# 0xJchen/HanabiZero

Measured on NVIDIA B200. Metric: mcts_simulations_per_sec, higher is better.
Workload: dtype f32

## Files before the change

hanabizero_b200/csrc/hz_rowchain.cu:

```cuda
#include <cuda.h>
#include <cuda_fp16.h>

#include <stdlib.h>
#include <string.h>

#include "hz_common.cuh"

namespace hz {

constexpr int kBM = 128, kBK = 64, kF = 512, kH = 256;
constexpr int kKB = kBM * kBK * 2;
constexpr int kActBytes = kBM * kF * 2;
constexpr int kWSlot = 256 * kBK * 2;
constexpr int kWSlots = 3;
constexpr int kOffW = kActBytes, kOffAux = kOffW + kWSlots * kWSlot;
constexpr int kAuxBytes = 128 + 1024;
constexpr int kRowSmem = kOffAux + kAuxBytes + 1024;
constexpr int kEpiWarps = 16, kEpiThreads = kEpiWarps * 32, kRowThreads = 64 + kEpiThreads;
constexpr int kMaxPhases = 10, kMaps = 10;
constexpr int kMapX0 = 7, kMapState = 8, kMapOut = 9;
constexpr unsigned kSpin = 1u << 26;

struct RowJob {
  int32_t map, n0, batch, num_k, a_kb, n, half;
  int32_t relu, dst_kb;
  int32_t res, res_off;
  int32_t gout, gb;
  int32_t kb1;
  const __half* bias;
};
struct RowPhase {
  int32_t njobs, after;
  int32_t a_wait, res_load;
  RowJob job[2];
};
struct alignas(64) RowParams {
  CUtensorMap maps[kMaps];
  RowPhase phase[kMaxPhases];
  int32_t n_phases, rows, row_blocks, p3;
  const __half* x0; int64_t ld_x0;
  const __half* w1a_t;
  __half* state;
  __half* out;
  unsigned long long* trace;
};

namespace rc {

__device__ __forceinline__ uint32_t smem_u32(const void* p) { return (uint32_t)__cvta_generic_to_shared(p); }
__device__ __forceinline__ void mbar_init(uint32_t bar, uint32_t count) {
  asm volatile("mbarrier.init.shared::cta.b64 [%0], %1;" ::"r"(bar), "r"(count) : "memory");
}
__device__ __forceinline__ void mbar_expect_tx(uint32_t bar, uint32_t bytes) {
  asm volatile("mbarrier.arrive.expect_tx.shared::cta.b64 _, [%0], %1;" ::"r"(bar), "r"(bytes) : "memory");
}
__device__ __forceinline__ void mbar_arrive(uint32_t bar) {
  asm volatile("mbarrier.arrive.shared::cta.b64 _, [%0];" ::"r"(bar) : "memory");
}
__device__ __forceinline__ void mbar_wait(uint32_t bar, uint32_t parity) {
  uint32_t done = 0;
  for (unsigned spin = 0; !done; ++spin) {
    asm volatile(
        "{\n\t.reg .pred p;\n\t"
        "mbarrier.try_wait.parity.shared::cta.b64 p, [%1], %2;\n\t"
        "selp.u32 %0, 1, 0, p;\n\t}"
        : "=r"(done) : "r"(bar), "r"(parity) : "memory");
    if (spin > kSpin) __trap();
  }
}
__device__ __forceinline__ void tma_load_3d(uint32_t dst, const CUtensorMap* map, uint32_t bar, int c0, int c1, int c2) {
  asm volatile(
      "cp.async.bulk.tensor.3d.shared::cta.global.mbarrier::complete_tx::bytes [%0], [%1, {%3, %4, %5}], [%2];"
      ::"r"(dst), "l"(map), "r"(bar), "r"(c0), "r"(c1), "r"(c2) : "memory");
}
__device__ __forceinline__ void tma_store_3d(const CUtensorMap* map, uint32_t src, int c0, int c1, int c2) {
  asm volatile(
      "cp.async.bulk.tensor.3d.global.shared::cta.bulk_group [%0, {%2, %3, %4}], [%1];"
      ::"l"(map), "r"(src), "r"(c0), "r"(c1), "r"(c2) : "memory");
}
__device__ __forceinline__ void tma_commit() { asm volatile("cp.async.bulk.commit_group;" ::: "memory"); }
__device__ __forceinline__ void tma_wait_read_all() { asm volatile("cp.async.bulk.wait_group.read 0;" ::: "memory"); }
__device__ __forceinline__ void tma_wait_all() { asm volatile("cp.async.bulk.wait_group 0;" ::: "memory"); }
__device__ __forceinline__ void tma_wait_all_but_last() { asm volatile("cp.async.bulk.wait_group 1;" ::: "memory"); }
__device__ __forceinline__ void tma_prefetch_desc(const CUtensorMap* map) {
  asm volatile("prefetch.tensormap [%0];" ::"l"(map) : "memory");
}
__device__ __forceinline__ void tc_fence_before() { asm volatile("tcgen05.fence::before_thread_sync;" ::: "memory"); }
__device__ __forceinline__ void tc_fence_after() { asm volatile("tcgen05.fence::after_thread_sync;" ::: "memory"); }
__device__ __forceinline__ void tc_commit(uint32_t bar) {
  asm volatile("tcgen05.commit.cta_group::1.mbarrier::arrive::one.shared::cluster.b64 [%0];" ::"r"(bar) : "memory");
}
__device__ __forceinline__ void tc_mma_f16(uint32_t tmem_d, uint64_t desc_a, uint64_t desc_b, uint32_t idesc,
                                           uint32_t accumulate) {
  asm volatile(
      "{\n\t.reg .pred p;\n\t"
      "setp.ne.b32 p, %4, 0;\n\t"
      "tcgen05.mma.cta_group::1.kind::f16 [%0], %1, %2, %3, p;\n\t}"
      ::"r"(tmem_d), "l"(desc_a), "l"(desc_b), "r"(idesc), "r"(accumulate) : "memory");
}
__device__ __forceinline__ void tc_ld16(uint32_t taddr, uint32_t* r) {
  asm volatile(
      "tcgen05.ld.sync.aligned.32x32b.x16.b32 "
      "{%0, %1, %2, %3, %4, %5, %6, %7, %8, %9, %10, %11, %12, %13, %14, %15}, [%16];"
      : "=r"(r[0]), "=r"(r[1]), "=r"(r[2]), "=r"(r[3]), "=r"(r[4]), "=r"(r[5]), "=r"(r[6]), "=r"(r[7]),
        "=r"(r[8]), "=r"(r[9]), "=r"(r[10]), "=r"(r[11]), "=r"(r[12]), "=r"(r[13]), "=r"(r[14]), "=r"(r[15])
      : "r"(taddr) : "memory");
}
__device__ __forceinline__ void tc_wait_ld() { asm volatile("tcgen05.wait::ld.sync.aligned;" ::: "memory"); }

__device__ __forceinline__ uint64_t umma_desc_k128(uint32_t saddr) {
  uint64_t d = 0;
  d |= (uint64_t)((saddr & 0x3ffffu) >> 4);
  d |= (uint64_t)1 << 16;
  d |= (uint64_t)(1024 >> 4) << 32;
  d |= (uint64_t)1 << 46;
  d |= (uint64_t)2 << 61;
  return d;
}
__device__ __forceinline__ bool elect_one() {
  uint32_t pred;
  asm volatile(
      "{\n\t.reg .pred p;\n\t"
      "elect.sync _|p, 0xffffffff;\n\t"
      "selp.u32 %0, 1, 0, p;\n\t}"
      : "=r"(pred));
  return pred != 0;
}
__device__ __forceinline__ void st_shared_v4(uint32_t addr, uint4 v) {
  asm volatile("st.shared.v4.u32 [%0], {%1, %2, %3, %4};" ::"r"(addr), "r"(v.x), "r"(v.y), "r"(v.z), "r"(v.w) : "memory");
}
__device__ __forceinline__ uint4 ld_shared_v4(uint32_t addr) {
  uint4 v;
  asm volatile("ld.shared.v4.u32 {%0, %1, %2, %3}, [%4];" : "=r"(v.x), "=r"(v.y), "=r"(v.z), "=r"(v.w) : "r"(addr) : "memory");
  return v;
}
__device__ __forceinline__ uint32_t act_off(int r, int ch) {
  return (uint32_t)((ch >> 3) * kKB + (r >> 3) * 1024 + (r & 7) * 128 + ((((ch & 7) ^ (r & 7))) << 4));
}
__device__ __forceinline__ void stamp(const RowParams& P, int phase, int slot) {
  if (P.trace) {
    unsigned long long t;
    asm volatile("mov.u64 %0, %%globaltimer;" : "=l"(t));
    P.trace[((size_t)blockIdx.x * kMaxPhases + phase) * 4 + slot] = t;
  }
}

}

using namespace rc;

__global__ void __launch_bounds__(kRowThreads, 1) k_row_chain(const __grid_constant__ RowParams P) {
  extern __shared__ uint8_t smem_raw[];
  const uint32_t base = (smem_u32(smem_raw) + 1023u) & ~1023u;
  const uint32_t act = base, wbase = base + kOffW, aux = base + kOffAux;
  auto w_full = [&](int s) { return aux + 8u * s; };
  auto w_empty = [&](int s) { return aux + 8u * (kWSlots + s); };
  auto acc_full = [&](int h) { return aux + 8u * (2 * kWSlots + h); };
  const uint32_t ready0 = aux + 8u * (2 * kWSlots + 2), ready1 = ready0 + 8u;
  const uint32_t a_full = ready1 + 8u;
  const uint32_t res_full = a_full + 8u;
  const uint32_t tmem_slot = res_full + 8u;
  const uint32_t sbias = aux + 128u;
  const int warp = __shfl_sync(0xffffffffu, (int)(threadIdx.x >> 5), 0), lane = threadIdx.x & 31;

  if (warp == 0 && lane == 0) {
    for (int s = 0; s < kWSlots; ++s) { mbar_init(w_full(s), 1); mbar_init(w_empty(s), 1); }
    mbar_init(acc_full(0), 1);
    mbar_init(acc_full(1), 1);
    mbar_init(ready0, kEpiWarps);
    mbar_init(ready1, kEpiWarps);
    mbar_init(a_full, 1);
    mbar_init(res_full, 1);
    asm volatile("fence.mbarrier_init.release.cluster;" ::: "memory");
    for (int m = 0; m < kMaps; ++m) tma_prefetch_desc(&P.maps[m]);
  }
  if (warp == 1) {
    asm volatile("tcgen05.alloc.cta_group::1.sync.aligned.shared::cta.b32 [%0], %1;" ::"r"(tmem_slot), "n"(512) : "memory");
    asm volatile("tcgen05.relinquish_alloc_permit.cta_group::1.sync.aligned;" ::: "memory");
  }
  tc_fence_before();
  __syncthreads();
  tc_fence_after();
  uint32_t tmem_base;
  asm volatile("ld.shared.u32 %0, [%1];" : "=r"(tmem_base) : "r"(tmem_slot) : "memory");

  if (warp == 0) {
    const bool leader = elect_one();
    uint32_t slot = 0, e_par = 0xffffffffu;
    for (int rb = blockIdx.x; rb < P.row_blocks; rb += gridDim.x) {
      for (int ph = 0; ph < P.n_phases; ++ph) {
        const RowPhase& F = P.phase[ph];
        for (int j = 0; j < F.njobs; ++j) {
          const RowJob& J = F.job[j];
          const uint32_t bytes = (uint32_t)J.n * (kBK * 2);
          for (int kb = 0; kb < J.num_k; ++kb) {
            mbar_wait(w_empty(slot), (e_par >> slot) & 1u);
            e_par ^= 1u << slot;
            if (leader) {
              mbar_expect_tx(w_full(slot), bytes);
              tma_load_3d(wbase + slot * kWSlot, &P.maps[J.map], w_full(slot), kb * kBK, J.n0, J.batch);
            }
            __syncwarp();
            if (++slot == kWSlots) slot = 0;
          }
        }
      }
    }
  } else if (warp == 1) {
    const bool leader = elect_one();
    uint32_t slot = 0, f_par = 0, r0_par = 0, r1_par = 0, af_par = 0;
    bool first_rb = true;
    for (int rb = blockIdx.x; rb < P.row_blocks; rb += gridDim.x) {
      for (int ph = 0; ph < P.n_phases; ++ph) {
        const RowPhase& F = P.phase[ph];
        mbar_wait(ready0, r0_par);
        r0_par ^= 1u;
        tc_fence_after();
        bool got1 = false;
        auto need_all = [&]() {
          mbar_wait(ready1, r1_par);
          r1_par ^= 1u;
          if (F.a_wait) {
            mbar_wait(a_full, af_par);
            af_par ^= 1u;
          }
          tc_fence_after();
          got1 = true;
        };
        if (leader && first_rb) stamp(P, ph, 0);
        for (int j = 0; j < F.njobs; ++j) {
          const RowJob& J = F.job[j];
          const uint32_t d_tmem = tmem_base + (uint32_t)J.half * 256u;
          const uint32_t idesc = (1u << 4) | ((uint32_t)(J.n >> 3) << 17) | ((uint32_t)(kBM >> 4) << 24);
          uint64_t da = umma_desc_k128(act + (uint32_t)J.a_kb * kKB);
          for (int kb = 0; kb < J.num_k; ++kb) {
            if (!got1 && (j > 0 || kb >= J.kb1)) need_all();
            mbar_wait(w_full(slot), (f_par >> slot) & 1u);
            f_par ^= 1u << slot;
            tc_fence_after();
            if (leader) {
              const uint64_t dw = umma_desc_k128(wbase + slot * kWSlot);
#pragma unroll
              for (int k16 = 0; k16 < kBK / 16; ++k16) {
                tc_mma_f16(d_tmem, da + (uint64_t)(2 * k16), dw + (uint64_t)(2 * k16), idesc, (kb | k16) != 0);
              }
              tc_commit(w_empty(slot));
            }
            __syncwarp();
            da += (uint64_t)(kKB >> 4);
            if (++slot == kWSlots) slot = 0;
          }
          if (leader) tc_commit(acc_full(J.half));
          __syncwarp();
        }
        if (!got1) need_all();
        if (leader && first_rb) stamp(P, ph, 1);
      }
      first_rb = false;
    }
  } else {
    const int q = warp & 3, part = (warp - 2) >> 2, et = threadIdx.x - 64;
    const int rloc = q * 32 + lane;
    uint32_t a_par = 0;
    bool first_rb = true;
    auto load_tile = [&](int map, int rb_, uint32_t bar) {
      mbar_expect_tx(bar, kActBytes);
#pragma unroll
      for (int kb = 0; kb < kF / kBK; ++kb) tma_load_3d(act + kb * kKB, &P.maps[map], bar, kb * kBK, rb_ * kBM, 0);
    };
    uint32_t rf_par = 0;
    if (et == 0) load_tile(kMapX0, blockIdx.x, a_full);
    __syncwarp();
    if (lane == 0) { mbar_arrive(ready0); mbar_arrive(ready1); }
    for (int rb = blockIdx.x; rb < P.row_blocks; rb += gridDim.x) {
      const int row = rb * kBM + rloc;
      const bool live = row < P.rows;
      for (int ph = 0; ph < P.n_phases; ++ph) {
        const RowPhase& F = P.phase[ph];
        if (et == 0) tma_wait_read_all();
        asm volatile("bar.sync 1, %0;" ::"n"(kEpiThreads) : "memory");
        {
          const int j = et >> 8, col = et & 255;
          if (j < F.njobs && col < F.job[j].n) {
            const unsigned short bv = __half_as_ushort(F.job[j].bias[col]);
            asm volatile("st.shared.u16 [%0], %1;" ::"r"(sbias + 2u * et), "h"(bv) : "memory");
          }
        }
        const __half* crow[2] = {nullptr, nullptr};
        uint4 ef0 = make_uint4(0, 0, 0, 0), ef1 = ef0;
#pragma unroll
        for (int j = 0; j < 2; ++j) {
          if (j >= F.njobs) continue;
          const RowJob& J = F.job[j];
          if (J.res == 1 && live) {
            const uint4* oh = reinterpret_cast<const uint4*>(P.x0 + (size_t)row * P.ld_x0 + kF);
            int a = -1;
#pragma unroll
            for (int v = 0; v < 4; ++v) {
              const uint4 w = oh[v];
              const uint32_t u[4] = {w.x, w.y, w.z, w.w};
#pragma unroll
              for (int t = 0; t < 4; ++t) {
                if ((u[t] & 0xffffu) == 0x3c00u) a = v * 8 + t * 2;
                if ((u[t] >> 16) == 0x3c00u) a = v * 8 + t * 2 + 1;
              }
            }
            if (a >= 0) crow[j] = P.w1a_t + (size_t)a * kF + J.res_off;
          } else if (J.res == 2 && live) {
            crow[j] = P.x0 + (size_t)row * P.ld_x0 + J.res_off;
          }
          if (j == 0 && crow[0]) {
            const int c0 = ((part * (J.n >> 4)) >> 2) * 16;
            ef0 = __ldg(reinterpret_cast<const uint4*>(crow[0] + c0));
            ef1 = __ldg(reinterpret_cast<const uint4*>(crow[0] + c0 + 8));
          }
        }
        asm volatile("bar.sync 1, %0;" ::"n"(kEpiThreads) : "memory");
        for (int j = 0; j < F.njobs; ++j) {
          const int h = F.job[j].half;
          mbar_wait(acc_full(h), (a_par >> h) & 1u);
          a_par ^= 1u << h;
        }
        tc_fence_after();
        if (et == 0 && first_rb) stamp(P, ph, 2);
        if (F.res_load) {
          if (et == 0) load_tile(kMapX0, rb, res_full);
          mbar_wait(res_full, rf_par);
          rf_par ^= 1u;
        }
        bool any_store = false;
#pragma unroll
        for (int j = 0; j < 2; ++j) {
          if (j >= F.njobs) continue;
          const RowJob& J = F.job[j];
          const int n16 = J.n >> 4;
          const int c_begin = ((part * n16) >> 2) * 16, c_end = (((part + 1) * n16) >> 2) * 16;
          const uint32_t t_addr = tmem_base + (uint32_t)J.half * 256u + ((uint32_t)(q * 32) << 16);
          const uint32_t sb = sbias + (uint32_t)j * 512u;
          const __half* cr = crow[j];
          const int res = J.res, relu = J.relu, dst_kb = J.dst_kb, res_off = J.res_off;
          any_store |= J.gout != 0;
          auto fetch_res = [&](int c, uint4& e0, uint4& e1) {
            if (res == 3) {
              const int ch = res_off * 8 + (c >> 3);
              e0 = ld_shared_v4(act + act_off(rloc, ch));
              e1 = ld_shared_v4(act + act_off(rloc, ch + 1));
            } else if (cr) {
              e0 = __ldg(reinterpret_cast<const uint4*>(cr + c));
              e1 = __ldg(reinterpret_cast<const uint4*>(cr + c + 8));
            }
          };
          auto emit = [&](const uint32_t (&r)[16], const uint4& e0, const uint4& e1, int c) {
            const uint4 b0 = ld_shared_v4(sb + 2u * (uint32_t)c), b1 = ld_shared_v4(sb + 2u * (uint32_t)c + 16u);
            float v[16];
            const __half2* h0 = reinterpret_cast<const __half2*>(&b0);
            const __half2* h1 = reinterpret_cast<const __half2*>(&b1);
#pragma unroll
            for (int t = 0; t < 4; ++t) {
              const float2 f0 = __half22float2(h0[t]), f1 = __half22float2(h1[t]);
              v[2 * t] = __uint_as_float(r[2 * t]) + f0.x;
              v[2 * t + 1] = __uint_as_float(r[2 * t + 1]) + f0.y;
              v[8 + 2 * t] = __uint_as_float(r[8 + 2 * t]) + f1.x;
              v[8 + 2 * t + 1] = __uint_as_float(r[8 + 2 * t + 1]) + f1.y;
            }
            if (res != 0) {
              const __half2* g0 = reinterpret_cast<const __half2*>(&e0);
              const __half2* g1 = reinterpret_cast<const __half2*>(&e1);
#pragma unroll
              for (int t = 0; t < 4; ++t) {
                const float2 x0 = __half22float2(g0[t]), x1 = __half22float2(g1[t]);
                v[2 * t] += x0.x; v[2 * t + 1] += x0.y; v[8 + 2 * t] += x1.x; v[8 + 2 * t + 1] += x1.y;
              }
            }
            uint4 o0, o1;
            __half2* p0 = reinterpret_cast<__half2*>(&o0);
            __half2* p1 = reinterpret_cast<__half2*>(&o1);
#pragma unroll
            for (int t = 0; t < 4; ++t) {
              p0[t] = __floats2half2_rn(v[2 * t], v[2 * t + 1]);
              p1[t] = __floats2half2_rn(v[8 + 2 * t], v[8 + 2 * t + 1]);
            }
            if (relu) {
              const __half2 z = __float2half2_rn(0.0f);
#pragma unroll
              for (int t = 0; t < 4; ++t) { p0[t] = __hmax2(p0[t], z); p1[t] = __hmax2(p1[t], z); }
            }
            if (dst_kb >= 0) {
              const int ch = dst_kb * 8 + (c >> 3);
              st_shared_v4(act + act_off(rloc, ch), o0);
              st_shared_v4(act + act_off(rloc, ch + 1), o1);
            }
          };
          uint32_t ra[16], rb2[16];
          uint4 ea0 = ef0, ea1 = ef1, eb0 = make_uint4(0, 0, 0, 0), eb1 = eb0;
          if (j == 1 || res == 3) {
            ea0 = ea1 = make_uint4(0, 0, 0, 0);
            fetch_res(c_begin, ea0, ea1);
          }
          tc_ld16(t_addr + (uint32_t)c_begin, ra);
          for (int c = c_begin; c < c_end; c += 32) {
            tc_wait_ld();
            const bool more1 = c + 16 < c_end;
            if (more1) {
              tc_ld16(t_addr + (uint32_t)(c + 16), rb2);
              if (res != 0) fetch_res(c + 16, eb0, eb1);
            }
            emit(ra, ea0, ea1, c);
            if (more1) {
              tc_wait_ld();
              if (c + 32 < c_end) {
                tc_ld16(t_addr + (uint32_t)(c + 32), ra);
                if (res != 0) fetch_res(c + 32, ea0, ea1);
              }
              emit(rb2, eb0, eb1, c + 16);
            }
          }
          if (j == 0) {
            asm volatile("fence.proxy.async.shared::cta;" ::: "memory");
            tc_fence_before();
            __syncwarp();
            if (lane == 0) mbar_arrive(ready0);
          }
        }
        if (any_store || F.after != 0) {
          asm volatile("fence.proxy.async.shared::cta;" ::: "memory");
          asm volatile("bar.sync 1, %0;" ::"n"(kEpiThreads) : "memory");
          if (et == 0) {
            for (int j = 0; j < F.njobs; ++j) {
              const RowJob& J = F.job[j];
              if (J.gout == 1 && j == 0) {
                for (int kb = 0; kb < kF / kBK; ++kb) tma_store_3d(&P.maps[kMapState], act + kb * kKB, kb * kBK, rb * kBM, 0);
              } else if (J.gout == 2) {
                for (int i = 0; i * kBK < P.p3; ++i)
                  tma_store_3d(&P.maps[kMapOut], act + (J.dst_kb + i) * kKB, i * kBK, rb * kBM, J.gb);
              }
            }
            if (any_store) tma_commit();
            if (F.after == 1) {
              tma_wait_all_but_last();
              tma_wait_read_all();
              asm volatile("fence.proxy.async;" ::: "memory");
              load_tile(kMapState, rb, a_full);
            } else if (F.after == 2 && rb + (int)gridDim.x < P.row_blocks) {
              tma_wait_read_all();
              load_tile(kMapX0, rb + gridDim.x, a_full);
            }
          }
        }
        if (et == 0 && first_rb) stamp(P, ph, 3);
        asm volatile("fence.proxy.async.shared::cta;" ::: "memory");
        tc_fence_before();
        __syncwarp();
        if (lane == 0) mbar_arrive(ready1);
      }
      first_rb = false;
    }
  }

  if (threadIdx.x == 64) tma_wait_all();
  tc_fence_before();
  __syncthreads();
  if (warp == 1) {
    asm volatile("tcgen05.dealloc.cta_group::1.sync.aligned.b32 %0, %1;" ::"r"(tmem_base), "n"(512) : "memory");
  }
}

typedef CUresult (*EncodeTiledFn)(CUtensorMap*, CUtensorMapDataType, cuuint32_t, void*, const cuuint64_t*,
                                  const cuuint64_t*, const cuuint32_t*, const cuuint32_t*, CUtensorMapInterleave,
                                  CUtensorMapSwizzle, CUtensorMapL2promotion, CUtensorMapFloatOOBfill);

static EncodeTiledFn encode_fn() {
  static EncodeTiledFn fn = [] {
    void* p = nullptr;
    cudaDriverEntryPointQueryResult q;
    if (cudaGetDriverEntryPoint("cuTensorMapEncodeTiled", &p, cudaEnableDefault, &q) != cudaSuccess ||
        q != cudaDriverEntryPointSuccess) {
      p = nullptr;
    }
    cudaGetLastError();
    return (EncodeTiledFn)p;
  }();
  return fn;
}

static bool make_w_map(CUtensorMap* map, const void* ptr, int64_t k, int64_t n, int64_t batch, int64_t ld, int box_n) {
  EncodeTiledFn fn = encode_fn();
  if (!fn) return false;
  cuuint64_t dims[3] = {(cuuint64_t)k, (cuuint64_t)n, (cuuint64_t)batch};
  cuuint64_t strides[2] = {(cuuint64_t)ld * 2, (cuuint64_t)(n * ld) * 2};
  cuuint32_t box[3] = {(cuuint32_t)kBK, (cuuint32_t)box_n, 1};
  cuuint32_t estr[3] = {1, 1, 1};
  return fn(map, CU_TENSOR_MAP_DATA_TYPE_FLOAT16, 3, const_cast<void*>(ptr), dims, strides, box, estr,
            CU_TENSOR_MAP_INTERLEAVE_NONE, CU_TENSOR_MAP_SWIZZLE_128B, CU_TENSOR_MAP_L2_PROMOTION_L2_256B,
            CU_TENSOR_MAP_FLOAT_OOB_FILL_NONE) == CUDA_SUCCESS;
}

}

using namespace hz;

struct hz_rowchain {
  int device = 0, grid = 0, sms = 0;
  RowParams params;
  unsigned long long* trace = nullptr;
};

extern "C" {
#pragma GCC visibility push(default)

int hz_rowchain_create(hz_rowchain** out, int device, const hz_rowchain_weights* w, int rows, const void* x0,
                       int64_t ld_x0, void* state, void* out_logits) {
  if (!out || !w || rows <= 0 || !x0 || !state || !out_logits) { set_error("hz_rowchain_create: bad argument"); return HZ_ERR_ARG; }
  if (w->state_cols != kF || w->head_cols != kH || w->onehot_cols != 32 || w->logit_cols <= 0 || w->logit_cols > 256 ||
      w->logit_cols % 16 || ld_x0 < kF + 32 || ld_x0 % 8 || w->ld_w1 < kF + 32 || w->ld_w1 % 8) {
    set_error("hz_rowchain_create: this executor is built for state 512 / heads 256 / one-hot 32 / logits <= 256 (multiple of 16)");
    return HZ_ERR_ARG;
  }
  const void* ptrs[] = {w->w1, w->w1a_t, w->b1, w->w2, w->b2, w->w3, w->b3, w->wh1, w->bh1, w->wb2, w->bb2,
                        w->wa2, w->ba2, w->wb3, w->bb3, x0, state, out_logits};
  for (const void* p : ptrs) {
    if (!p || ((uintptr_t)p & 15)) { set_error("hz_rowchain_create: null or unaligned pointer"); return HZ_ERR_ARG; }
  }
  DeviceGuard dg(device);
  if (!dg.ok) { set_error("hz_rowchain_create: cannot select device %d", device); return HZ_ERR_CUDA; }
  if (!encode_fn()) { set_error("hz_rowchain_create: cuTensorMapEncodeTiled unavailable"); return HZ_ERR_CUDA; }
  hz_rowchain* e = new hz_rowchain;
  e->device = device;
  RowParams& P = e->params;
  memset(&P, 0, sizeof(P));
  const int p3 = w->logit_cols;
  bool ok = make_w_map(&P.maps[0], w->w1, kF, kF, 1, w->ld_w1, 256) &&
            make_w_map(&P.maps[1], w->w2, kF, kF, 1, kF, 256) &&
            make_w_map(&P.maps[2], w->w3, kF, kF, 1, kF, 256) &&
            make_w_map(&P.maps[3], w->wh1, kF, 3 * kH, 1, kF, 256) &&
            make_w_map(&P.maps[4], w->wb2, kH, kH, 3, kH, 256) &&
            make_w_map(&P.maps[5], w->wa2, kH, kH, 1, kH, 256) &&
            make_w_map(&P.maps[6], w->wb3, kH, p3, 3, kH, p3) &&
            make_w_map(&P.maps[kMapX0], x0, kF, rows, 1, ld_x0, kBM) &&
            make_w_map(&P.maps[kMapState], state, kF, rows, 1, kF, kBM) &&
            make_w_map(&P.maps[kMapOut], out_logits, p3, rows, 3, p3, kBM);
  if (!ok) { delete e; set_error("hz_rowchain_create: cuTensorMapEncodeTiled failed"); return HZ_ERR_CUDA; }
  const __half *b1 = (const __half*)w->b1, *b2 = (const __half*)w->b2, *b3 = (const __half*)w->b3,
               *bh1 = (const __half*)w->bh1, *bb2 = (const __half*)w->bb2, *ba2 = (const __half*)w->ba2,
               *bb3 = (const __half*)w->bb3;
  auto job = [](int map, int n0, int batch, int num_k, int a_kb, int n, int half, const __half* bias, int relu,
                int dst_kb, int res = 0, int res_off = 0, int gout = 0, int gb = 0) {
    RowJob j;
    memset(&j, 0, sizeof(j));
    j.map = map; j.n0 = n0; j.batch = batch; j.num_k = num_k; j.a_kb = a_kb; j.n = n; j.half = half;
    j.bias = bias; j.relu = relu; j.dst_kb = dst_kb; j.res = res; j.res_off = res_off; j.gout = gout; j.gb = gb;
    return j;
  };
  int np = 0;
  auto phase = [&](int after, RowJob j0, const RowJob* j1 = nullptr, int a_wait = 0) {
    RowPhase& F = P.phase[np++];
    F.after = after; F.njobs = j1 ? 2 : 1; F.job[0] = j0; F.a_wait = a_wait;
    if (j1) F.job[1] = *j1;
  };
  RowJob t;
  t = job(0, 256, 0, 8, 0, 256, 1, b1 + 256, 1, 4, 1, 256);  phase(0, job(0, 0, 0, 8, 0, 256, 0, b1, 1, 0, 1, 0), &t, 1);
  t = job(1, 256, 0, 8, 0, 256, 1, b2 + 256, 1, 4);          phase(0, job(1, 0, 0, 8, 0, 256, 0, b2, 1, 0), &t);
  t = job(2, 256, 0, 8, 0, 256, 1, b3 + 256, 1, 4, 3, 4, 1);
  phase(0, job(2, 0, 0, 8, 0, 256, 0, b3, 1, 0, 3, 0, 1), &t);
  P.phase[np - 1].res_load = 1;
  t = job(3, 512, 0, 8, 0, 256, 1, bh1 + 512, 1, 4);         phase(0, job(3, 256, 0, 8, 0, 256, 0, bh1 + 256, 1, 0), &t);
  t = job(4, 0, 2, 4, 4, 256, 1, bb2 + 512, 1, 4);           phase(0, job(4, 0, 1, 4, 0, 256, 0, bb2 + 256, 1, 0), &t);
  t = job(6, 0, 1, 4, 4, p3, 1, bb3 + p3, 0, 4, 0, 0, 2, 1);
  phase(1, job(6, 0, 0, 4, 0, p3, 0, bb3, 0, 0, 0, 0, 2, 0), &t);
  phase(0, job(3, 0, 0, 8, 0, 256, 0, bh1, 1, 0), nullptr, 1);
  phase(0, job(4, 0, 0, 4, 0, 256, 1, bb2, 1, 4));
  phase(0, job(5, 0, 0, 4, 4, 256, 0, ba2, 1, 0, 3, 0));
  phase(2, job(6, 0, 2, 4, 0, p3, 1, bb3 + 2 * p3, 0, 4, 0, 0, 2, 2));
  for (int p = 0; p < np; ++p) {
    RowPhase& F = P.phase[p];
    F.job[0].kb1 = 0;
    F.job[1].kb1 = 0;
    if (p == 0 || F.a_wait) continue;
    const RowJob& A = P.phase[p - 1].job[0];
    RowJob& J = F.job[0];
    if (J.half != A.half || A.dst_kb < 0 || P.phase[p - 1].after != 0) continue;
    const int w0 = (A.n + kBK - 1) / kBK;
    int k = 0;
    while (k < J.num_k && J.a_kb + k >= A.dst_kb && J.a_kb + k < A.dst_kb + w0) ++k;
    J.kb1 = k;
  }
  P.n_phases = np;
  P.rows = rows;
  P.row_blocks = (rows + kBM - 1) / kBM;
  P.p3 = p3;
  P.x0 = (const __half*)x0;
  P.ld_x0 = ld_x0;
  P.w1a_t = (const __half*)w->w1a_t;
  P.state = (__half*)state;
  P.out = (__half*)out_logits;
  cudaError_t err = cudaFuncSetAttribute(k_row_chain, cudaFuncAttributeMaxDynamicSharedMemorySize, kRowSmem);
  cudaDeviceProp prop;
  if (err == cudaSuccess) err = cudaGetDeviceProperties(&prop, device);
  if (err != cudaSuccess) { delete e; return fail_cuda(err, "hz_rowchain_create: setup"); }
  e->sms = prop.multiProcessorCount;
  e->grid = P.row_blocks < e->sms ? P.row_blocks : e->sms;
  *out = e;
  return HZ_OK;
}

int hz_rowchain_destroy(hz_rowchain* e) {
  if (!e) return HZ_OK;
  DeviceGuard dg(e->device);
  if (e->trace) cudaFree(e->trace);
  delete e;
  return HZ_OK;
}

int hz_rowchain_set_state(hz_rowchain* e, void* state) {
  if (!e || !state || ((uintptr_t)state & 15)) { set_error("hz_rowchain_set_state: bad argument"); return HZ_ERR_ARG; }
  if (state == (void*)e->params.state) return HZ_OK;
  if (!make_w_map(&e->params.maps[kMapState], state, kF, e->params.rows, 1, kF, kBM)) {
    set_error("hz_rowchain_set_state: cuTensorMapEncodeTiled failed");
    return HZ_ERR_CUDA;
  }
  e->params.state = (__half*)state;
  return HZ_OK;
}

int hz_rowchain_set_trace(hz_rowchain* e, int enable) {
  if (!e) { set_error("hz_rowchain_set_trace: bad argument"); return HZ_ERR_ARG; }
  DeviceGuard dg(e->device);
  if (enable && !e->trace) {
    const size_t bytes = (size_t)e->sms * kMaxPhases * 4 * sizeof(unsigned long long);
    HZ_CUDA(cudaMalloc(&e->trace, bytes));
    HZ_CUDA(cudaMemset(e->trace, 0, bytes));
  }
  e->params.trace = enable ? e->trace : nullptr;
  return HZ_OK;
}

int hz_rowchain_read_trace(hz_rowchain* e, uint64_t* host_out, int64_t count) {
  if (!e || !e->trace || !host_out || count <= 0) { set_error("hz_rowchain_read_trace: no trace"); return HZ_ERR_ARG; }
  DeviceGuard dg(e->device);
  const int64_t have = (int64_t)e->grid * kMaxPhases * 4;
  HZ_CUDA(cudaMemcpy(host_out, e->trace, (size_t)(count < have ? count : have) * sizeof(uint64_t), cudaMemcpyDeviceToHost));
  return HZ_OK;
}

int hz_rowchain_grid(const hz_rowchain* e) { return e ? e->grid : 0; }

int hz_rowchain_run(hz_rowchain* e, void* stream) {
  if (!e) { set_error("hz_rowchain_run: bad argument"); return HZ_ERR_ARG; }
  DeviceGuard dg(e->device);
  k_row_chain<<<e->grid, kRowThreads, kRowSmem, (cudaStream_t)stream>>>(e->params);
  HZ_LAUNCH_CHECK("k_row_chain");
  return HZ_OK;
}

#pragma GCC visibility pop
}
```

Before: 177.9 million.

## Run row-chain MLP as 2-CTA cluster pairs with cta_group::2 MMA and smem action table

```diff
diff --git a/hanabizero_b200/csrc/hz_rowchain.cu b/hanabizero_b200/csrc/hz_rowchain.cu
--- a/hanabizero_b200/csrc/hz_rowchain.cu
+++ b/hanabizero_b200/csrc/hz_rowchain.cu
@@ -11,14 +11,15 @@
 constexpr int kBM = 128, kBK = 64, kF = 512, kH = 256;
 constexpr int kKB = kBM * kBK * 2;
 constexpr int kActBytes = kBM * kF * 2;
-constexpr int kWSlot = 256 * kBK * 2;
-constexpr int kWSlots = 3;
-constexpr int kOffW = kActBytes, kOffAux = kOffW + kWSlots * kWSlot;
+constexpr int kWSlot = 128 * kBK * 2;
+constexpr int kWSlots = 4;
+constexpr int kActions = 32, kTabBytes = kActions * kF * 2;
+constexpr int kOffW = kActBytes, kOffTab = kOffW + kWSlots * kWSlot, kOffAux = kOffTab + kTabBytes;
 constexpr int kAuxBytes = 128 + 1024;
 constexpr int kRowSmem = kOffAux + kAuxBytes + 1024;
 constexpr int kEpiWarps = 16, kEpiThreads = kEpiWarps * 32, kRowThreads = 64 + kEpiThreads;
-constexpr int kMaxPhases = 10, kMaps = 10;
-constexpr int kMapX0 = 7, kMapState = 8, kMapOut = 9;
+constexpr int kMaxPhases = 10, kMaps = 11;
+constexpr int kMapX0 = 7, kMapState = 8, kMapOut = 9, kMapTab = 10;
 constexpr unsigned kSpin = 1u << 26;
 
 struct RowJob {
@@ -39,7 +40,6 @@
   RowPhase phase[kMaxPhases];
   int32_t n_phases, rows, row_blocks, p3;
   const __half* x0; int64_t ld_x0;
-  const __half* w1a_t;
   __half* state;
   __half* out;
   unsigned long long* trace;
@@ -68,10 +68,46 @@
     if (spin > kSpin) __trap();
   }
 }
+__device__ __forceinline__ void mbar_wait_cluster(uint32_t bar, uint32_t parity) {
+  uint32_t done = 0;
+  for (unsigned spin = 0; !done; ++spin) {
+    asm volatile(
+        "{\n\t.reg .pred p;\n\t"
+        "mbarrier.try_wait.parity.acquire.cluster.shared::cta.b64 p, [%1], %2;\n\t"
+        "selp.u32 %0, 1, 0, p;\n\t}"
+        : "=r"(done) : "r"(bar), "r"(parity) : "memory");
+    if (spin > kSpin) __trap();
+  }
+}
+__device__ __forceinline__ uint32_t lead_addr(uint32_t addr) {
+  uint32_t r;
+  asm volatile("mapa.shared::cluster.u32 %0, %1, 0;" : "=r"(r) : "r"(addr));
+  return r;
+}
+__device__ __forceinline__ void mbar_arrive_lead(uint32_t bar) {
+  asm volatile("mbarrier.arrive.shared::cluster.b64 _, [%0];" ::"r"(lead_addr(bar)) : "memory");
+}
+__device__ __forceinline__ void mbar_expect_tx_lead(uint32_t bar, uint32_t bytes) {
+  asm volatile("mbarrier.arrive.expect_tx.shared::cluster.b64 _, [%0], %1;" ::"r"(lead_addr(bar)), "r"(bytes)
+               : "memory");
+}
+__device__ __forceinline__ void cluster_sync() {
+  asm volatile("barrier.cluster.arrive.release.aligned;\n\tbarrier.cluster.wait.acquire.aligned;" ::: "memory");
+}
+__device__ __forceinline__ uint32_t cluster_rank() {
+  uint32_t r;
+  asm volatile("mov.u32 %0, %%cluster_ctarank;" : "=r"(r));
+  return r;
+}
 __device__ __forceinline__ void tma_load_3d(uint32_t dst, const CUtensorMap* map, uint32_t bar, int c0, int c1, int c2) {
   asm volatile(
       "cp.async.bulk.tensor.3d.shared::cta.global.mbarrier::complete_tx::bytes [%0], [%1, {%3, %4, %5}], [%2];"
       ::"r"(dst), "l"(map), "r"(bar), "r"(c0), "r"(c1), "r"(c2) : "memory");
+}
+__device__ __forceinline__ void tma_load_3d_lead(uint32_t dst, const CUtensorMap* map, uint32_t bar, int c0, int c1, int c2) {
+  asm volatile(
+      "cp.async.bulk.tensor.3d.shared::cluster.global.mbarrier::complete_tx::bytes.cta_group::2 [%0], [%1, {%3, %4, %5}], [%2];"
+      ::"r"(dst), "l"(map), "r"(lead_addr(bar)), "r"(c0), "r"(c1), "r"(c2) : "memory");
 }
 __device__ __forceinline__ void tma_store_3d(const CUtensorMap* map, uint32_t src, int c0, int c1, int c2) {
   asm volatile(
@@ -87,15 +123,16 @@
 }
 __device__ __forceinline__ void tc_fence_before() { asm volatile("tcgen05.fence::before_thread_sync;" ::: "memory"); }
 __device__ __forceinline__ void tc_fence_after() { asm volatile("tcgen05.fence::after_thread_sync;" ::: "memory"); }
-__device__ __forceinline__ void tc_commit(uint32_t bar) {
-  asm volatile("tcgen05.commit.cta_group::1.mbarrier::arrive::one.shared::cluster.b64 [%0];" ::"r"(bar) : "memory");
+__device__ __forceinline__ void tc_commit_pair(uint32_t bar) {
+  asm volatile("tcgen05.commit.cta_group::2.mbarrier::arrive::one.shared::cluster.multicast::cluster.b64 [%0], %1;"
+               ::"r"(bar), "h"((unsigned short)3) : "memory");
 }
 __device__ __forceinline__ void tc_mma_f16(uint32_t tmem_d, uint64_t desc_a, uint64_t desc_b, uint32_t idesc,
                                            uint32_t accumulate) {
   asm volatile(
       "{\n\t.reg .pred p;\n\t"
       "setp.ne.b32 p, %4, 0;\n\t"
-      "tcgen05.mma.cta_group::1.kind::f16 [%0], %1, %2, %3, p;\n\t}"
+      "tcgen05.mma.cta_group::2.kind::f16 [%0], %1, %2, %3, p;\n\t}"
       ::"r"(tmem_d), "l"(desc_a), "l"(desc_b), "r"(idesc), "r"(accumulate) : "memory");
 }
 __device__ __forceinline__ void tc_ld16(uint32_t taddr, uint32_t* r) {
@@ -137,11 +174,14 @@
 __device__ __forceinline__ uint32_t act_off(int r, int ch) {
   return (uint32_t)((ch >> 3) * kKB + (r >> 3) * 1024 + (r & 7) * 128 + ((((ch & 7) ^ (r & 7))) << 4));
 }
-__device__ __forceinline__ void stamp(const RowParams& P, int phase, int slot) {
+__device__ __forceinline__ uint32_t tab_off(int a, int ch) {
+  return (uint32_t)((ch >> 3) * (kActions * 128) + a * 128 + ((((ch & 7) ^ (a & 7))) << 4));
+}
+__device__ __forceinline__ void stamp(const RowParams& P, int cta, int phase, int slot) {
   if (P.trace) {
     unsigned long long t;
     asm volatile("mov.u64 %0, %%globaltimer;" : "=l"(t));
-    P.trace[((size_t)blockIdx.x * kMaxPhases + phase) * 4 + slot] = t;
+    P.trace[((size_t)cta * kMaxPhases + phase) * 4 + slot] = t;
   }
 }
 
@@ -152,34 +192,38 @@
 __global__ void __launch_bounds__(kRowThreads, 1) k_row_chain(const __grid_constant__ RowParams P) {
   extern __shared__ uint8_t smem_raw[];
   const uint32_t base = (smem_u32(smem_raw) + 1023u) & ~1023u;
-  const uint32_t act = base, wbase = base + kOffW, aux = base + kOffAux;
+  const uint32_t act = base, wbase = base + kOffW, tab = base + kOffTab, aux = base + kOffAux;
   auto w_full = [&](int s) { return aux + 8u * s; };
   auto w_empty = [&](int s) { return aux + 8u * (kWSlots + s); };
   auto acc_full = [&](int h) { return aux + 8u * (2 * kWSlots + h); };
   const uint32_t ready0 = aux + 8u * (2 * kWSlots + 2), ready1 = ready0 + 8u;
   const uint32_t a_full = ready1 + 8u;
   const uint32_t res_full = a_full + 8u;
-  const uint32_t tmem_slot = res_full + 8u;
+  const uint32_t tab_full = res_full + 8u;
+  const uint32_t tmem_slot = tab_full + 8u;
   const uint32_t sbias = aux + 128u;
   const int warp = __shfl_sync(0xffffffffu, (int)(threadIdx.x >> 5), 0), lane = threadIdx.x & 31;
+  const int rank = (int)cluster_rank();
+  const int pairs = (P.row_blocks + 1) >> 1, grid_pairs = (int)gridDim.x >> 1;
 
   if (warp == 0 && lane == 0) {
     for (int s = 0; s < kWSlots; ++s) { mbar_init(w_full(s), 1); mbar_init(w_empty(s), 1); }
     mbar_init(acc_full(0), 1);
     mbar_init(acc_full(1), 1);
-    mbar_init(ready0, kEpiWarps);
-    mbar_init(ready1, kEpiWarps);
-    mbar_init(a_full, 1);
+    mbar_init(ready0, 2 * kEpiWarps);
+    mbar_init(ready1, 2 * kEpiWarps);
+    mbar_init(a_full, 2);
     mbar_init(res_full, 1);
+    mbar_init(tab_full, 1);
     asm volatile("fence.mbarrier_init.release.cluster;" ::: "memory");
     for (int m = 0; m < kMaps; ++m) tma_prefetch_desc(&P.maps[m]);
   }
   if (warp == 1) {
-    asm volatile("tcgen05.alloc.cta_group::1.sync.aligned.shared::cta.b32 [%0], %1;" ::"r"(tmem_slot), "n"(512) : "memory");
-    asm volatile("tcgen05.relinquish_alloc_permit.cta_group::1.sync.aligned;" ::: "memory");
+    asm volatile("tcgen05.alloc.cta_group::2.sync.aligned.shared::cta.b32 [%0], %1;" ::"r"(tmem_slot), "n"(512) : "memory");
+    asm volatile("tcgen05.relinquish_alloc_permit.cta_group::2.sync.aligned;" ::: "memory");
   }
   tc_fence_before();
-  __syncthreads();
+  cluster_sync();
   tc_fence_after();
   uint32_t tmem_base;
   asm volatile("ld.shared.u32 %0, [%1];" : "=r"(tmem_base) : "r"(tmem_slot) : "memory");
@@ -187,18 +231,18 @@
   if (warp == 0) {
     const bool leader = elect_one();
     uint32_t slot = 0, e_par = 0xffffffffu;
-    for (int rb = blockIdx.x; rb < P.row_blocks; rb += gridDim.x) {
+    for (int pr = (int)blockIdx.x >> 1; pr < pairs; pr += grid_pairs) {
       for (int ph = 0; ph < P.n_phases; ++ph) {
         const RowPhase& F = P.phase[ph];
         for (int j = 0; j < F.njobs; ++j) {
           const RowJob& J = F.job[j];
-          const uint32_t bytes = (uint32_t)J.n * (kBK * 2);
+          const int n0 = J.n0 + rank * (J.n >> 1);
           for (int kb = 0; kb < J.num_k; ++kb) {
             mbar_wait(w_empty(slot), (e_par >> slot) & 1u);
             e_par ^= 1u << slot;
             if (leader) {
-              mbar_expect_tx(w_full(slot), bytes);
-              tma_load_3d(wbase + slot * kWSlot, &P.maps[J.map], w_full(slot), kb * kBK, J.n0, J.batch);
+              if (rank == 0) mbar_expect_tx(w_full(slot), (uint32_t)J.n * (kBK * 2));
+              tma_load_3d_lead(wbase + slot * kWSlot, &P.maps[J.map], w_full(slot), kb * kBK, n0, J.batch);
             }
             __syncwarp();
             if (++slot == kWSlots) slot = 0;
@@ -207,31 +251,31 @@
       }
     }
   } else if (warp == 1) {
-    const bool leader = elect_one();
+    const bool leader = elect_one() && rank == 0;
     uint32_t slot = 0, f_par = 0, r0_par = 0, r1_par = 0, af_par = 0;
     bool first_rb = true;
-    for (int rb = blockIdx.x; rb < P.row_blocks; rb += gridDim.x) {
+    for (int pr = (int)blockIdx.x >> 1; rank == 0 && pr < pairs; pr += grid_pairs) {
       for (int ph = 0; ph < P.n_phases; ++ph) {
         const RowPhase& F = P.phase[ph];
-        mbar_wait(ready0, r0_par);
+        mbar_wait_cluster(ready0, r0_par);
         r0_par ^= 1u;
         tc_fence_after();
         bool got1 = false;
         auto need_all = [&]() {
-          mbar_wait(ready1, r1_par);
+          mbar_wait_cluster(ready1, r1_par);
           r1_par ^= 1u;
           if (F.a_wait) {
-            mbar_wait(a_full, af_par);
+            mbar_wait_cluster(a_full, af_par);
             af_par ^= 1u;
           }
           tc_fence_after();
           got1 = true;
         };
-        if (leader && first_rb) stamp(P, ph, 0);
+        if (leader && first_rb) { stamp(P, blockIdx.x, ph, 0); stamp(P, blockIdx.x + 1, ph, 0); }
         for (int j = 0; j < F.njobs; ++j) {
           const RowJob& J = F.job[j];
           const uint32_t d_tmem = tmem_base + (uint32_t)J.half * 256u;
-          const uint32_t idesc = (1u << 4) | ((uint32_t)(J.n >> 3) << 17) | ((uint32_t)(kBM >> 4) << 24);
+          const uint32_t idesc = (1u << 4) | ((uint32_t)(J.n >> 3) << 17) | ((uint32_t)((2 * kBM) >> 4) << 24);
           uint64_t da = umma_desc_k128(act + (uint32_t)J.a_kb * kKB);
           for (int kb = 0; kb < J.num_k; ++kb) {
             if (!got1 && (j > 0 || kb >= J.kb1)) need_all();
@@ -244,17 +288,17 @@
               for (int k16 = 0; k16 < kBK / 16; ++k16) {
                 tc_mma_f16(d_tmem, da + (uint64_t)(2 * k16), dw + (uint64_t)(2 * k16), idesc, (kb | k16) != 0);
               }
-              tc_commit(w_empty(slot));
+              tc_commit_pair(w_empty(slot));
             }
             __syncwarp();
             da += (uint64_t)(kKB >> 4);
             if (++slot == kWSlots) slot = 0;
           }
-          if (leader) tc_commit(acc_full(J.half));
+          if (leader) tc_commit_pair(acc_full(J.half));
           __syncwarp();
         }
         if (!got1) need_all();
-        if (leader && first_rb) stamp(P, ph, 1);
+        if (leader && first_rb) { stamp(P, blockIdx.x, ph, 1); stamp(P, blockIdx.x + 1, ph, 1); }
       }
       first_rb = false;
     }
@@ -263,16 +307,29 @@
     const int rloc = q * 32 + lane;
     uint32_t a_par = 0;
     bool first_rb = true;
-    auto load_tile = [&](int map, int rb_, uint32_t bar) {
-      mbar_expect_tx(bar, kActBytes);
-#pragma unroll
-      for (int kb = 0; kb < kF / kBK; ++kb) tma_load_3d(act + kb * kKB, &P.maps[map], bar, kb * kBK, rb_ * kBM, 0);
+    auto load_tile = [&](int map, int rb_, bool for_mma) {
+      if (for_mma) {
+        mbar_expect_tx_lead(a_full, kActBytes);
+#pragma unroll
+        for (int kb = 0; kb < kF / kBK; ++kb) tma_load_3d_lead(act + kb * kKB, &P.maps[map], a_full, kb * kBK, rb_ * kBM, 0);
+      } else {
+        mbar_expect_tx(res_full, kActBytes);
+#pragma unroll
+        for (int kb = 0; kb < kF / kBK; ++kb) tma_load_3d(act + kb * kKB, &P.maps[map], res_full, kb * kBK, rb_ * kBM, 0);
+      }
     };
     uint32_t rf_par = 0;
-    if (et == 0) load_tile(kMapX0, blockIdx.x, a_full);
+    if (et == 0) {
+      load_tile(kMapX0, blockIdx.x, true);
+      mbar_expect_tx(tab_full, kTabBytes);
+#pragma unroll
+      for (int kb = 0; kb < kF / kBK; ++kb) tma_load_3d(tab + kb * (kActions * 128), &P.maps[kMapTab], tab_full, kb * kBK, 0, 0);
+    }
     __syncwarp();
-    if (lane == 0) { mbar_arrive(ready0); mbar_arrive(ready1); }
-    for (int rb = blockIdx.x; rb < P.row_blocks; rb += gridDim.x) {
+    if (lane == 0) { mbar_arrive_lead(ready0); mbar_arrive_lead(ready1); }
+    mbar_wait(tab_full, 0);
+    for (int pr = (int)blockIdx.x >> 1; pr < pairs; pr += grid_pairs) {
+      const int rb = 2 * pr + rank;
       const int row = rb * kBM + rloc;
       const bool live = row < P.rows;
       for (int ph = 0; ph < P.n_phases; ++ph) {
@@ -288,25 +345,25 @@
         }
         const __half* crow[2] = {nullptr, nullptr};
         uint4 ef0 = make_uint4(0, 0, 0, 0), ef1 = ef0;
+        int act_row = -1;
+        if (F.job[0].res == 1 && live) {
+          const uint4* oh = reinterpret_cast<const uint4*>(P.x0 + (size_t)row * P.ld_x0 + kF);
+#pragma unroll
+          for (int v = 0; v < 4; ++v) {
+            const uint4 w = oh[v];
+            const uint32_t u[4] = {w.x, w.y, w.z, w.w};
+#pragma unroll
+            for (int t = 0; t < 4; ++t) {
+              if ((u[t] & 0xffffu) == 0x3c00u) act_row = v * 8 + t * 2;
+              if ((u[t] >> 16) == 0x3c00u) act_row = v * 8 + t * 2 + 1;
+            }
+          }
+        }
 #pragma unroll
         for (int j = 0; j < 2; ++j) {
           if (j >= F.njobs) continue;
           const RowJob& J = F.job[j];
-          if (J.res == 1 && live) {
-            const uint4* oh = reinterpret_cast<const uint4*>(P.x0 + (size_t)row * P.ld_x0 + kF);
-            int a = -1;
-#pragma unroll
-            for (int v = 0; v < 4; ++v) {
-              const uint4 w = oh[v];
-              const uint32_t u[4] = {w.x, w.y, w.z, w.w};
-#pragma unroll
-              for (int t = 0; t < 4; ++t) {
-                if ((u[t] & 0xffffu) == 0x3c00u) a = v * 8 + t * 2;
-                if ((u[t] >> 16) == 0x3c00u) a = v * 8 + t * 2 + 1;
-              }
-            }
-            if (a >= 0) crow[j] = P.w1a_t + (size_t)a * kF + J.res_off;
-          } else if (J.res == 2 && live) {
+          if (J.res == 2 && live) {
             crow[j] = P.x0 + (size_t)row * P.ld_x0 + J.res_off;
           }
           if (j == 0 && crow[0]) {
@@ -322,9 +379,9 @@
           a_par ^= 1u << h;
         }
         tc_fence_after();
-        if (et == 0 && first_rb) stamp(P, ph, 2);
+        if (et == 0 && first_rb) stamp(P, blockIdx.x, ph, 2);
         if (F.res_load) {
-          if (et == 0) load_tile(kMapX0, rb, res_full);
+          if (et == 0) load_tile(kMapX0, rb, false);
           mbar_wait(res_full, rf_par);
           rf_par ^= 1u;
         }
@@ -345,6 +402,12 @@
               const int ch = res_off * 8 + (c >> 3);
               e0 = ld_shared_v4(act + act_off(rloc, ch));
               e1 = ld_shared_v4(act + act_off(rloc, ch + 1));
+            } else if (res == 1) {
+              if (act_row >= 0) {
+                const int ch = (res_off + c) >> 3;
+                e0 = ld_shared_v4(tab + tab_off(act_row, ch));
+                e1 = ld_shared_v4(tab + tab_off(act_row, ch + 1));
+              }
             } else if (cr) {
               e0 = __ldg(reinterpret_cast<const uint4*>(cr + c));
               e1 = __ldg(reinterpret_cast<const uint4*>(cr + c + 8));
@@ -393,7 +456,7 @@
           };
           uint32_t ra[16], rb2[16];
           uint4 ea0 = ef0, ea1 = ef1, eb0 = make_uint4(0, 0, 0, 0), eb1 = eb0;
-          if (j == 1 || res == 3) {
+          if (j == 1 || res != 2) {
             ea0 = ea1 = make_uint4(0, 0, 0, 0);
             fetch_res(c_begin, ea0, ea1);
           }
@@ -419,7 +482,7 @@
             asm volatile("fence.proxy.async.shared::cta;" ::: "memory");
             tc_fence_before();
             __syncwarp();
-            if (lane == 0) mbar_arrive(ready0);
+            if (lane == 0) mbar_arrive_lead(ready0);
           }
         }
         if (any_store || F.after != 0) {
@@ -440,18 +503,18 @@
               tma_wait_all_but_last();
               tma_wait_read_all();
               asm volatile("fence.proxy.async;" ::: "memory");
-              load_tile(kMapState, rb, a_full);
-            } else if (F.after == 2 && rb + (int)gridDim.x < P.row_blocks) {
+              load_tile(kMapState, rb, true);
+            } else if (F.after == 2 && pr + grid_pairs < pairs) {
               tma_wait_read_all();
-              load_tile(kMapX0, rb + gridDim.x, a_full);
-            }
-          }
-        }
-        if (et == 0 && first_rb) stamp(P, ph, 3);
+              load_tile(kMapX0, rb + (int)gridDim.x, true);
+            }
+          }
+        }
+        if (et == 0 && first_rb) stamp(P, blockIdx.x, ph, 3);
         asm volatile("fence.proxy.async.shared::cta;" ::: "memory");
         tc_fence_before();
         __syncwarp();
-        if (lane == 0) mbar_arrive(ready1);
+        if (lane == 0) mbar_arrive_lead(ready1);
       }
       first_rb = false;
     }
@@ -459,9 +522,10 @@
 
   if (threadIdx.x == 64) tma_wait_all();
   tc_fence_before();
-  __syncthreads();
+  cluster_sync();
   if (warp == 1) {
-    asm volatile("tcgen05.dealloc.cta_group::1.sync.aligned.b32 %0, %1;" ::"r"(tmem_base), "n"(512) : "memory");
+    tc_fence_after();
+    asm volatile("tcgen05.dealloc.cta_group::2.sync.aligned.b32 %0, %1;" ::"r"(tmem_base), "n"(512) : "memory");
   }
 }
 
@@ -505,6 +569,21 @@
   unsigned long long* trace = nullptr;
 };
 
+static void row_launch_config(cudaLaunchConfig_t& cfg, cudaLaunchAttribute& attr, int grid, cudaStream_t stream) {
+  memset(&cfg, 0, sizeof(cfg));
+  memset(&attr, 0, sizeof(attr));
+  attr.id = cudaLaunchAttributeClusterDimension;
+  attr.val.clusterDim.x = 2;
+  attr.val.clusterDim.y = 1;
+  attr.val.clusterDim.z = 1;
+  cfg.gridDim = dim3((unsigned)grid);
+  cfg.blockDim = dim3(kRowThreads);
+  cfg.dynamicSmemBytes = kRowSmem;
+  cfg.stream = stream;
+  cfg.attrs = &attr;
+  cfg.numAttrs = 1;
+}
+
 extern "C" {
 #pragma GCC visibility push(default)
 
@@ -529,13 +608,14 @@
   RowParams& P = e->params;
   memset(&P, 0, sizeof(P));
   const int p3 = w->logit_cols;
-  bool ok = make_w_map(&P.maps[0], w->w1, kF, kF, 1, w->ld_w1, 256) &&
-            make_w_map(&P.maps[1], w->w2, kF, kF, 1, kF, 256) &&
-            make_w_map(&P.maps[2], w->w3, kF, kF, 1, kF, 256) &&
-            make_w_map(&P.maps[3], w->wh1, kF, 3 * kH, 1, kF, 256) &&
-            make_w_map(&P.maps[4], w->wb2, kH, kH, 3, kH, 256) &&
-            make_w_map(&P.maps[5], w->wa2, kH, kH, 1, kH, 256) &&
-            make_w_map(&P.maps[6], w->wb3, kH, p3, 3, kH, p3) &&
+  bool ok = make_w_map(&P.maps[0], w->w1, kF, kF, 1, w->ld_w1, 128) &&
+            make_w_map(&P.maps[1], w->w2, kF, kF, 1, kF, 128) &&
+            make_w_map(&P.maps[2], w->w3, kF, kF, 1, kF, 128) &&
+            make_w_map(&P.maps[3], w->wh1, kF, 3 * kH, 1, kF, 128) &&
+            make_w_map(&P.maps[4], w->wb2, kH, kH, 3, kH, 128) &&
+            make_w_map(&P.maps[5], w->wa2, kH, kH, 1, kH, 128) &&
+            make_w_map(&P.maps[6], w->wb3, kH, p3, 3, kH, p3 / 2) &&
+            make_w_map(&P.maps[kMapTab], w->w1a_t, kF, kActions, 1, kF, kActions) &&
             make_w_map(&P.maps[kMapX0], x0, kF, rows, 1, ld_x0, kBM) &&
             make_w_map(&P.maps[kMapState], state, kF, rows, 1, kF, kBM) &&
             make_w_map(&P.maps[kMapOut], out_logits, p3, rows, 3, p3, kBM);
@@ -590,7 +670,6 @@
   P.p3 = p3;
   P.x0 = (const __half*)x0;
   P.ld_x0 = ld_x0;
-  P.w1a_t = (const __half*)w->w1a_t;
   P.state = (__half*)state;
   P.out = (__half*)out_logits;
   cudaError_t err = cudaFuncSetAttribute(k_row_chain, cudaFuncAttributeMaxDynamicSharedMemorySize, kRowSmem);
@@ -598,7 +677,17 @@
   if (err == cudaSuccess) err = cudaGetDeviceProperties(&prop, device);
   if (err != cudaSuccess) { delete e; return fail_cuda(err, "hz_rowchain_create: setup"); }
   e->sms = prop.multiProcessorCount;
-  e->grid = P.row_blocks < e->sms ? P.row_blocks : e->sms;
+  cudaLaunchConfig_t cfg;
+  cudaLaunchAttribute attr;
+  row_launch_config(cfg, attr, 2 * ((P.row_blocks + 1) / 2), nullptr);
+  int max_pairs = 0;
+  err = cudaOccupancyMaxActiveClusters(&max_pairs, k_row_chain, &cfg);
+  if (err != cudaSuccess || max_pairs <= 0) {
+    delete e;
+    return fail_cuda(err != cudaSuccess ? err : cudaErrorInvalidConfiguration, "hz_rowchain_create: no CTA pair fits");
+  }
+  const int pairs = (P.row_blocks + 1) / 2;
+  e->grid = 2 * (pairs < max_pairs ? pairs : max_pairs);
   *out = e;
   return HZ_OK;
 }
@@ -647,7 +736,10 @@
 int hz_rowchain_run(hz_rowchain* e, void* stream) {
   if (!e) { set_error("hz_rowchain_run: bad argument"); return HZ_ERR_ARG; }
   DeviceGuard dg(e->device);
-  k_row_chain<<<e->grid, kRowThreads, kRowSmem, (cudaStream_t)stream>>>(e->params);
+  cudaLaunchConfig_t cfg;
+  cudaLaunchAttribute attr;
+  row_launch_config(cfg, attr, e->grid, (cudaStream_t)stream);
+  cudaLaunchKernelEx(&cfg, k_row_chain, e->params);
   HZ_LAUNCH_CHECK("k_row_chain");
   return HZ_OK;
 }
```

Result: no change. 178.0 million, median of 6 (+0.1%).
